# smarterclayton/kubernetes

Measured on AMD Instinct MI355X. Metric: pods scheduled/sec, higher is better.
Workload: dtype int64; 1 GPU; config2: 5000 nodes, 1776000 pods, DefaultProvider; nodes=5000, prefix_pods=0, placed_in_prefix=0, parallelism=speculative windows: all-CU snapshot scoring + in-order exact resolver

## Files before the change

### kubernetes_amd/csrc/ksg_plain.hip

```cpp
#include "ksg_launch.h"
#include "ksg_resolver.h"
#include "ksg_score.h"

#define KSG_NCAND 6
#define KSG_CSV_MAX 10
#define KSG_NO_CAND 7u
#define KSG_CSNAP 10
#define KSG_XR_W 20
#ifndef KSG_PL_PROD_SLEEP
#define KSG_PL_PROD_SLEEP 1
#endif
#ifndef KSG_PL_CHK_SLEEP
#define KSG_PL_CHK_SLEEP 2
#endif
#ifndef KSG_PL_XN_SLEEP
#define KSG_PL_XN_SLEEP 0
#endif
__host__ __device__ constexpr uint32_t pl_nt(int P) { return P >= 32 ? 512u : 768u; }
#define KSG_PL_FW KSG_RES_P0
#define KSG_PL_P0 (KSG_PL_FW + 1)
__host__ __device__ constexpr bool pl_d1(uint32_t P) { return P <= 4; }

struct alignas(16) PlCommit {
  uint32_t kind;
  uint32_t slot;
  uint32_t node;
  uint32_t flags;
  int32_t out;
  uint32_t xn;
  uint32_t pad[2];
};
struct alignas(16) PlCtl {
  uint32_t stop;
  uint32_t resolved;
  uint32_t sel_seq;
  uint32_t n_peer;
  uint32_t chk_seq[KSG_RES_NCHK];
  uint32_t chk_cnt[KSG_RES_NCHK][2];
  uint32_t chk_msk[KSG_RES_NCHK][2][2];
  uint32_t fin[KSG_RES_NCHK];
  uint32_t hang;
  uint32_t bad;
  uint32_t xseq;
  uint32_t xres[2];
  uint32_t xn_seq;
  uint32_t fin_x;
  uint32_t t_x, t_n;
  uint32_t fseq;
  uint32_t fin_f;
  uint32_t chk_rmsk[KSG_RES_NCHK][2][2];
  uint32_t chk_jmsk[KSG_RES_NCHK][2][2];
  uint32_t chk_nmsk[KSG_RES_NCHK][2][2];
  int32_t xsig[2];
};
struct PlLdsOff {
  uint32_t ctl, r_hdr, r_t0, r_wp, r_lp, r_rec, r_mod, r_svc, r_cand, r_csnap, r_csv, r_d1;
  uint32_t clist, xrow, dpos, sig, cm, peer, pub, drw, flag, peerset;
  uint32_t total;
};

__host__ __device__ inline PlLdsOff plain_lds_offsets(uint32_t P, uint32_t nflag, uint32_t W) {
  PlLdsOff o;
  const uint32_t R = win2_ring(P, false);
  uint32_t at = 0;
  o.ctl = at;     at += win_al16(sizeof(PlCtl));
  o.r_hdr = at;   at += win_al16((size_t)R * sizeof(RingHdr));
  o.r_t0 = at;    at += win_al16((size_t)R * P * 64 * 8);
  o.r_wp = at;    at += win_al16((size_t)R * P * 64 * 2);
  o.r_lp = at;    at += win_al16((size_t)R * 32 * 8);
  o.r_rec = at;   at += win_al16((size_t)R * KSG_WIN_SUM_DWORDS * 4);
  o.r_mod = at;   at += win_al16((size_t)R * 64 * 4);
  o.r_svc = at;   at += win_al16((size_t)R * sizeof(RingSvc));
  o.r_cand = at;  at += win_al16((size_t)R * 8 * 4);
  o.r_csnap = at; at += win_al16((size_t)R * KSG_NCAND * KSG_CSNAP * 8);
  o.r_csv = at;   at += win_al16((size_t)R * KSG_NCAND * KSG_SLOT_SVCS * 4);
  o.r_d1 = at;    at += pl_d1(P) ? win_al16((size_t)R * P * 64 * 8) : 0u;
  o.clist = at;   at += win_al16((size_t)KSG_MAX_SLOTS * KSG_CL_W * 4);
  o.xrow = at;    at += win_al16((size_t)KSG_MAX_SLOTS * KSG_XR_W * 4);
  o.dpos = at;    at += win_al16((size_t)2 * KSG_MAX_SLOTS * 4);
  o.sig = at;     at += win_al16((size_t)2 * KSG_MAX_SLOTS * 4);
  o.cm = at;      at += win_al16((size_t)W * sizeof(PlCommit));
  o.peer = at;    at += win_al16((size_t)win_peer_cap(nflag, W) * 2 * 4);
  o.pub = at;     at += win_al16((size_t)((W + 31) / 32) * 4);
  o.drw = at;     at += win_al16((size_t)((W + 31) / 32) * 4);
  o.flag = at;    at += win_al16((size_t)nflag * 4);
// ... 192 lines not shown
  for (int k = 0; k < 8; ++k) s += (uint32_t)__builtin_amdgcn_readlane((int)v, k);
  return s >= fused_group_arrivals(g, nwg, (uint32_t)pl_pg(P));
}

template <int P, bool STAMP, bool XS, bool FUSED>
__device__ __forceinline__ void win_plain_body(const KsgDev d, uint32_t wcap, KsgWinRun* run,
                                               const KsgWinSum* __restrict__ sums, const KsgWinXchg x,
                                               uint64_t* rng_io, int32_t* __restrict__ out_batch, const KsgFused f) {
  extern __shared__ __attribute__((aligned(16))) char smem[];
  uint32_t t_blk0 = 0;
  if constexpr (FUSED) {
    if (blockIdx.x != 0) {
      fused_score_blocks<P, STAMP>(d, wcap, run, sums, x, f, smem);
      return;
    }
    if constexpr (STAMP) t_blk0 = (uint32_t)__builtin_amdgcn_s_memrealtime();
  }
  KsgWinRun* const run_out = FUSED ? f.run_out : run;
  const uint32_t pos = run->pos, n_batch = run->n;
  if (run->halt || pos >= n_batch) {
    if (FUSED && threadIdx.x == 0) *run_out = *run;
    return;
  }
  if (FUSED && STAMP && threadIdx.x == 0 && d.dbgbuf)
    __hip_atomic_store(d.dbgbuf + 55, (int32_t)t_blk0, __ATOMIC_RELAXED, __HIP_MEMORY_SCOPE_AGENT);
  const uint32_t n_pods = min(wcap, n_batch - pos);
  int32_t* __restrict__ out = out_batch + pos;
  const uint32_t tid = threadIdx.x;
  const uint32_t lane = tid & 63;
  const uint32_t wave = __builtin_amdgcn_readfirstlane(tid >> 6);
  const uint32_t nflag = (d.n_services + 31) / 32;
  constexpr uint32_t RING = win2_ring(P, false);
  constexpr uint32_t NT = pl_nt(P);
  constexpr uint32_t NPW = NT / 64 - KSG_PL_P0;
  const uint32_t f_nwg = FUSED ? (d.nwords + NT / 64 - 1) / (NT / 64) : 0u;
  constexpr uint32_t DW = KSG_WIN_SUM_DWORDS;
  const PlLdsOff o = plain_lds_offsets(P, nflag, wcap);
  PlCtl* ctl = reinterpret_cast<PlCtl*>(smem + o.ctl);
  RingHdr* r_hdr = reinterpret_cast<RingHdr*>(smem + o.r_hdr);
  uint64_t* r_t0 = reinterpret_cast<uint64_t*>(smem + o.r_t0);
  uint64_t* r_d1 = reinterpret_cast<uint64_t*>(smem + o.r_d1);
  uint16_t* r_wp = reinterpret_cast<uint16_t*>(smem + o.r_wp);
  uint32_t* r_lp = reinterpret_cast<uint32_t*>(smem + o.r_lp);
  uint32_t* r_rec = reinterpret_cast<uint32_t*>(smem + o.r_rec);
  uint32_t* r_mod = reinterpret_cast<uint32_t*>(smem + o.r_mod);
  RingSvc* r_svc = reinterpret_cast<RingSvc*>(smem + o.r_svc);
  uint32_t* r_cand = reinterpret_cast<uint32_t*>(smem + o.r_cand);
  uint64_t* r_csnap = reinterpret_cast<uint64_t*>(smem + o.r_csnap);
  int32_t* r_csv = reinterpret_cast<int32_t*>(smem + o.r_csv);
  PlCommit* L_cm = reinterpret_cast<PlCommit*>(smem + o.cm);
  uint32_t* L_peer = reinterpret_cast<uint32_t*>(smem + o.peer);
  uint32_t* L_flag = reinterpret_cast<uint32_t*>(smem + o.flag);
  uint32_t* L_peerset = reinterpret_cast<uint32_t*>(smem + o.peerset);
  uint32_t* L_pub = reinterpret_cast<uint32_t*>(smem + o.pub);
  uint32_t* L_drw = reinterpret_cast<uint32_t*>(smem + o.drw);
  uint32_t* L_cl = reinterpret_cast<uint32_t*>(smem + o.clist);
  uint32_t* L_xr = reinterpret_cast<uint32_t*>(smem + o.xrow);
  uint32_t* L_dpos = reinterpret_cast<uint32_t*>(smem + o.dpos);
  int32_t* L_sig = reinterpret_cast<int32_t*>(smem + o.sig);
  const bool spread_on = d.w_spread != 0;
  const bool aff_on = (d.preds & KSG_PRED_SERVICEAFFINITY) && d.n_aff > 0;
  const bool res_on = (d.preds & KSG_PRED_PODFITSRESOURCES) != 0;
  const bool ports_on = (d.preds & KSG_PRED_PODFITSPORTS) != 0;
  const bool disk_on = (d.preds & KSG_PRED_NODISKCONFLICT) != 0;
  const bool xs_on = XS && (d.ext_filters & KSG_EXT_SCALAR) && d.n_scalar > 0;
  const bool esc = XS && x.esc != 0;
  const uint32_t nbits = (wcap + 31) / 32;
  const uint32_t skew = STAMP ? ((uint32_t)d.dbg >> 16) & 15u : 0u;
  const uint32_t xpt = STAMP ? ((uint32_t)d.dbg >> 24) & 15u : 0u;

  for (uint32_t t = tid; t < RING; t += NT) r_hdr[t].ready = 0;
  if (tid == 0) *ctl = PlCtl{};
  if constexpr (FUSED)
    for (uint32_t t = tid; t < f.ngroups * 8u; t += NT) st_mut(f.cnt + (size_t)(f.set ^ 1u) * f.ngroups * 8u + t, 0u);
  for (uint32_t w = tid; w < nflag; w += NT) {
    L_flag[w] = 0;
    L_peerset[w] = 0;
  }
  for (uint32_t w = tid; w < nbits; w += NT) {
    L_pub[w] = 0;
    L_drw[w] = 0;
  }
  __syncthreads();
  const uint64_t rng0 = *rng_io;

  if (wave >= KSG_PL_P0) {
    const uint32_t* recs = reinterpret_cast<const uint32_t*>(sums);
    uint64_t p_last = 0, p_acc = 0;
    auto pstamp = [&](uint32_t k) {
      if constexpr (STAMP) {
        const uint64_t t_now = __builtin_amdgcn_s_memtime();
        p_acc += lane == k ? t_now - p_last : 0ULL;
        p_last = t_now;
      }
    };
    if constexpr (STAMP) p_last = __builtin_amdgcn_s_memtime();
    const uint64_t f_t0 = (STAMP && FUSED) ? __builtin_amdgcn_s_memrealtime() : 0ULL;
    uint64_t f_tg = 0;
    for (uint32_t j = wave - KSG_PL_P0; j < n_pods; j += NPW) {
      const uint32_t e = j % RING;
      for (uint32_t spin = 0;; ++spin) {
        if (ld_acq(&ctl->stop)) return;
        if (spin > KSG_SPIN_LIMIT) {
          ctl->hang = 1;
          return;
        }
        uint32_t done = min(ld_acq(&ctl->xseq), ld_acq(&ctl->fseq) + 2u);
#pragma unroll
        for (int c = 0; c < KSG_RES_NCHK; ++c) done = min(done, ld_acq(&ctl->chk_seq[c]));
        if (j < RING || done + RING >= j + 3) break;
        __builtin_amdgcn_s_sleep(KSG_PL_PROD_SLEEP);
      }
      pstamp(24);
      if (skew & 8u) __builtin_amdgcn_s_sleep(8);
      uint32_t rec, lpv, k0;
      int32_t m0;
      if constexpr (FUSED) {
        const uint32_t g = j / (uint32_t)pl_pg(P);
        const uint32_t g_lo = (j > 0 && j % (uint32_t)pl_pg(P) == 0) ? g - 1u : g;
        for (uint32_t spin = 0;; ++spin) {
          if (ld_acq(&ctl->stop)) return;
          if (spin > KSG_SPIN_LIMIT) {
            ctl->hang = 1;
            return;
          }
          if (fused_group_done<P>(f, g, f_nwg) && (g_lo == g || fused_group_done<P>(f, g_lo, f_nwg))) break;
          __builtin_amdgcn_s_sleep(1);
        }
        rec = lane < DW ? ld_mut(recs + (size_t)j * DW + lane) : 0u;
        const int32_t* pm = reinterpret_cast<const int32_t*>(x.buf + (size_t)x.wcap * x.ostride * 8) + (size_t)j * x.ostride;
        const uint64_t* pb = reinterpret_cast<const uint64_t*>(x.buf) + (size_t)j * x.ostride;
        const uint64_t* pd = reinterpret_cast<const uint64_t*>(x.buf + x.d1_off) + (size_t)j * x.ostride;
        int32_t mw[P];
        int32_t lm = KSG_S32_NONE;
        constexpr bool ONE = P <= 8;
        uint64_t b1[ONE ? P : 1];
#pragma unroll
        for (uint32_t q = 0; q < P; ++q) {
          const uint32_t wq = q * 64 + lane;
          mw[q] = wq < d.nwords ? ld_mut(pm + wq) : KSG_S32_NONE;
          if constexpr (ONE) b1[q] = wq < d.nwords ? ld_mut(pb + wq) : 0ULL;
          lm = mw[q] > lm ? mw[q] : lm;
        }
// ... 208 lines not shown
      const bool h_prev_s = h_d1 && pod_has_service(h_prv, h_s);
      const uint32_t h_pfl = (drawable ? 0u : 1u) | (h_prev_s ? 2u : 0u) | (h_over ? 4u : 0u) | (min(nk, 255u) << 8) |
                             (min(n_svcs, 255u) << 16) | (min(n_sel, 255u) << 24);
      if (lane == 0) {
        r_hdr[e].ps = h_s;
        r_hdr[e].pfl = h_pfl;
        r_hdr[e].psoft = e_ps;
        r_hdr[e].tmax = e_tm;
        r_hdr[e].tcnt = e_tc;
        r_hdr[e].m0 = m0;
        r_hdr[e].k0 = k0;
        r_hdr[e].r = r;
        r_hdr[e].drawable = drawable;
        r_hdr[e].pred = (int32_t)cand0;
        r_hdr[e].pad = csv_on ? 1u : 0u;
        st_rel(&r_hdr[e].ready, j + 1);
      }
      if constexpr (STAMP && FUSED) {
        if (j == 0 && lane == 0 && d.dbgbuf) {
          const uint64_t t_r = __builtin_amdgcn_s_memrealtime();
          atomicAdd(d.dbgbuf + 52, (int32_t)(f_tg - f_t0));
          atomicAdd(d.dbgbuf + 53, (int32_t)(t_r - f_tg));
          atomicAdd(d.dbgbuf + 54, 1);
        }
      }
      pstamp(27);
    }
    if constexpr (STAMP) {
      if (d.dbgbuf && lane >= 24 && lane < 28) atomicAdd(d.dbgbuf + lane, (int32_t)(p_acc / 64));
    }
    return;
  }

  if (wave >= KSG_RES_C0 && wave < KSG_RES_C0 + KSG_RES_NCHK) {
    __builtin_amdgcn_s_setprio(2);
    const uint32_t c = wave - KSG_RES_C0;
    const uint32_t my_slot = c * 64 + lane;
    const uint32_t* my_cl = L_cl + (size_t)my_slot * KSG_CL_W;
    RegSlot S;
    S.node = ~0u;
    S.cap_c = S.cap_m = S.snp_c = S.snp_m = S.dl_c = S.dl_m = 0;
    S.inv_c = S.inv_m = 0.0;
    S.nk = S.ns = S.smask = 0;
    S.row = ~0u;
    S.xk = 0;
    S.sst = 0;
    S.ntm = 0;
#pragma unroll
    for (int r = 0; r < 4; ++r) S.xh[r] = S.xdl[r] = 0;
    auto apply_v = [&](uint32_t p, uint4 cmv, uint32_t prec_v) {
      const uint32_t kind = __builtin_amdgcn_readfirstlane(cmv.x);
      const uint32_t slot = __builtin_amdgcn_readfirstlane(cmv.y);
      if (kind != 1 || (slot >> 6) != c) return;
      const uint32_t woff = __builtin_amdgcn_readfirstlane(cmv.z);
      const uint32_t fl = __builtin_amdgcn_readfirstlane(cmv.w);
      const bool fresh = (fl & 1u) != 0;
      const uint32_t cidx = (fl >> 1) & 7u, n_svcs = (fl >> 8) & 0xffu, bns = (fl >> 16) & 0xffu, bnk = fl >> 24;
      const uint32_t ol = slot & 63, ep = p % RING, wn = d.lo + woff;
      const uint32_t prec = lane < DW ? prec_v : 0u;
      const PodView ppv = pod_view(prec);
      if (fresh && lane == ol) {
        if (cidx < KSG_NCAND) {
          const uint64_t* cs = r_csnap + (ep * KSG_NCAND + cidx) * KSG_CSNAP;
          S.cap_c = (int64_t)cs[0];
          S.cap_m = (int64_t)cs[1];
          S.snp_c = (int64_t)cs[2];
          S.snp_m = (int64_t)cs[3];
          S.inv_c = __longlong_as_double((long long)cs[4]);
          S.inv_m = __longlong_as_double((long long)cs[5]);
// ... 31 lines not shown
        const bool staged = cidx < KSG_NCAND && r_hdr[ep].pad != 0;
        int32_t cnt = 0;
        if (sv_lane)
          cnt = staged ? r_csv[(ep * KSG_NCAND + cidx) * KSG_SLOT_SVCS + lane] : gld(d.svc_cnt + (size_t)sv * d.n_nodes + wn);
        if (sv_lane) L_cl[(size_t)slot * KSG_CL_W + KSG_CL_SC + bns + lane] = (uint32_t)cnt;
        new_mask = wave_or_u32(sv_lane ? (1u << (sv & 31)) : 0u);
      }
      if (lane == ol) {
        S.dl_c = (int64_t)((uint64_t)S.dl_c + (uint64_t)ppv.req_c);
        S.dl_m = (int64_t)((uint64_t)S.dl_m + (uint64_t)ppv.req_m);
        S.nk = bnk + ppv.nk;
        S.ns = bns + n_svcs;
        S.smask |= new_mask;
        if (XS) {
          S.xk |= ppv.xm;
#pragma unroll
          for (int r = 0; r < 4; ++r) S.xdl[r] += (int32_t)__builtin_amdgcn_readlane(prec, WS_XREQ + r);
        }
      }
    };
    auto apply = [&](uint32_t p) {
      apply_v(p, *reinterpret_cast<const uint4*>(&L_cm[p]), r_rec[(p % RING) * DW + min(lane, DW - 1)]);
    };

    uint64_t t_last = 0, t_acc = 0;
    auto cstamp = [&](uint32_t k) {
      if constexpr (STAMP) {
        const uint64_t t_now = __builtin_amdgcn_s_memtime();
        t_acc += lane == k ? t_now - t_last : 0ULL;
        t_last = t_now;
      }
    };
    if constexpr (STAMP) t_last = __builtin_amdgcn_s_memtime();
    for (uint32_t i = 0;; ++i) {
      const uint32_t e = i % RING, par = i & 1;
      bool stopped = false;
      for (uint32_t spin = 0;; ++spin) {
        const uint32_t ss = ld_rlx(&ctl->sel_seq), rd = ld_rlx(&r_hdr[e].ready), st = ld_rlx(&ctl->stop);
        if (i < n_pods && ss + 1 >= i && rd == i + 1) break;
        if (st) {
          stopped = true;
          break;
        }
        if (spin > 16 * KSG_SPIN_LIMIT) {
          ctl->hang = 1;
          stopped = true;
          break;
        }
        if (KSG_PL_CHK_SLEEP) __builtin_amdgcn_s_sleep(KSG_PL_CHK_SLEEP);
      }
      acq_lds();
      cstamp(c == 0 ? 16 : 19);
      if (stopped) {
        const uint32_t R = __builtin_amdgcn_readfirstlane(ctl->resolved);
        for (uint32_t q = i >= 2 ? i - 2 : 0; q < R; ++q) apply(q);
        break;
      }
      if (skew & 4u) __builtin_amdgcn_s_sleep(8);
      if (xpt & 2u) {
        if (lane == 0) {
          ctl->chk_cnt[c][par] = 0;
          ctl->chk_msk[c][par][0] = ctl->chk_msk[c][par][1] = 0;
          st_post(&ctl->chk_seq[c], i + 1);
        }
        continue;
      }
      if (i >= 2) apply(i - 2);
      cstamp(c == 0 ? 17 : 20);
      const uint32_t rec = lane < DW ? r_rec[e * DW + lane] : 0u;
      const int32_t m0 = (int32_t)__builtin_amdgcn_readfirstlane(r_hdr[e].m0);
      uint64_t e_fw = 0;
      int32_t e_cs = 0;
      if (esc && S.node != ~0u) {
        e_fw = gld(efit_word(x, i, S.node >> 6));
        const int32_t ps = (int32_t)__builtin_amdgcn_readfirstlane(r_rec[e * DW + WS_SVC]);
        if (spread_on && ps >= 0) e_cs = gld(d.svc_cnt + (size_t)ps * d.n_nodes + d.lo + S.node);
      }
      bool drop = false;
      uint32_t dpos = 0;
      uint32_t est = 0;
      int32_t esig = 0;
      if (!__builtin_amdgcn_readlane(rec, WS_ERR) && m0 != KSG_S32_NONE && S.node != ~0u) {
        const PodView pv = pod_view(rec);
        const uint32_t wd = S.node >> 6;
        const uint64_t tw = r_t0[(size_t)e * P * 64 + wd];
        SlotRow R;
        R.load(my_cl);
        dpos = r_lp[e * 64 + (wd >> 6) * 2] + r_wp[(size_t)e * P * 64 + wd] +
               (uint32_t)__popcll(tw & ((1ULL << (S.node & 63)) - 1ULL));
        cstamp(c == 0 ? 22 : 40);
        if (esc) {
          const bool in_t0 = (tw >> (S.node & 63)) & 1ULL;
          const int64_t now_c = (int64_t)((uint64_t)S.snp_c + (uint64_t)S.dl_c);
          const int64_t now_m = (int64_t)((uint64_t)S.snp_m + (uint64_t)S.dl_m);
          bool unfit = false;
          if (res_on && !pv.zero_req)
            unfit = !((S.cap_c == 0 || S.cap_c - now_c >= pv.req_c) && (S.cap_m == 0 || S.cap_m - now_m >= pv.req_m));
          if (S.xk & pv.xm)
#pragma unroll
            for (int r = 0; r < 4; ++r) {
// ... 57 lines not shown
            const int32_t lr_snap =
                lr_win_nb(S.snp_c + pv.req_c, S.cap_c, S.inv_c) + lr_win_nb(S.snp_m + pv.req_m, S.cap_m, S.inv_m);
            drop |= (lr_now >> 1) != (lr_snap >> 1);
          }
          cstamp(c == 0 ? 23 : 40);
          if (!drop && pv.nk && S.nk)
            drop |= R.key_hit(S.nk, rec, pv.nk, pv.n_ports, ports_on, disk_on);
          if (!drop && spread_on && pv.s >= 0 && ((S.smask >> (pv.s & 31)) & 1u)) {
            int32_t delta = 0, snapc = 0;
            R.svc(S.ns, (uint32_t)pv.s, snapc, delta);
            if (delta)
              drop = frac10_i32(pv.smax - snapc - delta, pv.smax) != frac10_i32(pv.smax - snapc, pv.smax);
          }
        }
      }
      if (drop || (est & 4u)) L_dpos[par * KSG_MAX_SLOTS + my_slot] = dpos;
      if (est & 2u) L_sig[par * KSG_MAX_SLOTS + my_slot] = esig;
      const uint64_t dmsk = __ballot(drop);
      if (esc) {
        const uint64_t rm = __ballot((est & 2u) != 0), jm = __ballot((est & 4u) != 0), nm = __ballot((est & 8u) != 0);
        if (lane == 0) {
          ctl->chk_rmsk[c][par][0] = (uint32_t)rm;
          ctl->chk_rmsk[c][par][1] = (uint32_t)(rm >> 32);
          ctl->chk_jmsk[c][par][0] = (uint32_t)jm;
          ctl->chk_jmsk[c][par][1] = (uint32_t)(jm >> 32);
          ctl->chk_nmsk[c][par][0] = (uint32_t)nm;
          ctl->chk_nmsk[c][par][1] = (uint32_t)(nm >> 32);
        }
      }
      if (lane == 0) {
        ctl->chk_cnt[c][par] = (uint32_t)__popcll(dmsk);
        ctl->chk_msk[c][par][0] = (uint32_t)dmsk;
        ctl->chk_msk[c][par][1] = (uint32_t)(dmsk >> 32);
        st_post(&ctl->chk_seq[c], i + 1);
      }
      cstamp(c == 0 ? 18 : 21);
    }
    if (S.node != ~0u) {
      const uint32_t n = d.lo + S.node;
      d.used_cpu[n] = (int64_t)((uint64_t)S.snp_c + (uint64_t)S.dl_c);
      d.used_mem[n] = (int64_t)((uint64_t)S.snp_m + (uint64_t)S.dl_m);
      for (uint32_t a = 0; a < S.nk; ++a)
        __hip_atomic_fetch_or(d.keymap + (size_t)my_cl[KSG_CL_KEY + a] * d.nw + (n >> 6), 1ULL << (n & 63),
                              __ATOMIC_RELAXED, __HIP_MEMORY_SCOPE_AGENT);
      for (uint32_t a = 0; a < S.ns; ++a) {
        const uint32_t sa = my_cl[KSG_CL_SV + a];
        bool first = true;
        int32_t count = 0;
        for (uint32_t b = 0; b < S.ns; ++b) {
          if (my_cl[KSG_CL_SV + b] == sa) {
            if (b < a) first = false;
            ++count;
          }
        }
        __hip_atomic_fetch_add(d.svc_total + sa, 1, __ATOMIC_RELAXED, __HIP_MEMORY_SCOPE_AGENT);
        if (first) {
          const int32_t fin = (int32_t)my_cl[KSG_CL_SC + a] + count;
          d.svc_cnt[(size_t)sa * d.n_nodes + n] = fin;
          if (fin > 0)
            __hip_atomic_fetch_or(d.svc_bits + (size_t)sa * d.nw + (n >> 6), 1ULL << (n & 63), __ATOMIC_RELAXED,
                                  __HIP_MEMORY_SCOPE_AGENT);
          __hip_atomic_fetch_max(d.svc_max + sa, fin, __ATOMIC_RELAXED, __HIP_MEMORY_SCOPE_AGENT);
        }
      }
    }
    if constexpr (STAMP) {
      if (d.dbgbuf && ((lane >= 16 && lane < 24) || lane == 9 || lane == 14 || lane == 15))
        atomicAdd(d.dbgbuf + lane, (int32_t)(t_acc / 64));
    }
    drain_stores();
    if (lane == 0) st_rel(&ctl->fin[c], 1u);
    return;
  }

  auto flags = [&](uint32_t q, uint32_t node, uint32_t cidx, uint32_t slot, uint32_t bns, uint32_t prec) {
    const uint32_t nss = __builtin_amdgcn_readlane(prec, WS_NSS), npp = __builtin_amdgcn_readlane(prec, WS_NPP);
    const uint32_t n_svcs = nss >> 16, n_sel = nss & 0xffff, pnk = (npp & 0xffff) + (npp >> 16);
    if (!n_svcs) return;
    const uint32_t wn = d.lo + node, eq = q % RING;
    const bool sv_lane = lane < n_svcs;
    const uint32_t my_sv =
        (uint32_t)__shfl((int)prec, (int)min(WS_IDS + pnk + n_sel + (sv_lane ? lane : 0u), 63u), 64);
    const bool staged = cidx < KSG_NCAND && r_hdr[eq].pad != 0;
    int32_t mx = 0, peer = 0, cnt = 0;
    if (sv_lane) {
      cnt = staged ? r_csv[(eq * KSG_NCAND + cidx) * KSG_SLOT_SVCS + lane] : gld(d.svc_cnt + (size_t)my_sv * d.n_nodes + wn);
      mx = r_svc[eq].max[lane];
      peer = r_svc[eq].peer[lane];
    }
    const uint32_t ent = lane - KSG_CL_SV < bns ? L_cl[(size_t)slot * KSG_CL_W + lane] : ~0u;
    uint32_t before = 0;
    for (uint32_t t = 0; t < n_svcs; ++t) {
      const uint32_t sv_t = (uint32_t)__builtin_amdgcn_readlane((int)my_sv, (int)t);
      const uint32_t b_t = (uint32_t)__popcll(__ballot(ent == sv_t));
      if (lane == t) before = b_t;
    }
    bool changed = sv_lane && aff_on && peer == -1 && !((L_peerset[my_sv >> 5] >> (my_sv & 31)) & 1u);
    uint64_t pm = __ballot(sv_lane && peer == -1);
    if (pm) {
      uint32_t n_peer = __builtin_amdgcn_readfirstlane(ctl->n_peer);
      while (pm) {
        const uint32_t b = __builtin_ctzll(pm);
        pm &= pm - 1;
        const uint32_t fsv = (uint32_t)__builtin_amdgcn_readlane((int)my_sv, (int)b);
        if (!((L_peerset[fsv >> 5] >> (fsv & 31)) & 1u)) {
          if (lane == 0) {
            L_peerset[fsv >> 5] |= 1u << (fsv & 31);
            L_peer[2 * n_peer] = fsv;
            L_peer[2 * n_peer + 1] = wn;
          }
          ++n_peer;
          lds_fence();
        }
      }
      if (lane == 0) ctl->n_peer = n_peer;
    }
    if (sv_lane && spread_on && cnt + (int32_t)before + 1 > mx) changed = true;
    if (changed) atomicOr(&L_flag[my_sv >> 5], 1u << (my_sv & 31));
  };
  if (wave == KSG_PL_FW) {
    auto flag_commit = [&](uint32_t q) {
      const uint4 cmv = *reinterpret_cast<const uint4*>(&L_cm[q]);
      if (__builtin_amdgcn_readfirstlane(cmv.x) != 1) return;
      const uint32_t slot = __builtin_amdgcn_readfirstlane(cmv.y), node = __builtin_amdgcn_readfirstlane(cmv.z);
      const uint32_t fl = __builtin_amdgcn_readfirstlane(cmv.w);
      const uint32_t prec = lane < DW ? r_rec[(q % RING) * DW + lane] : 0u;
      flags(q, node, (fl >> 1) & 7u, slot, (fl >> 16) & 0xffu, prec);
    };
    uint64_t f_last = 0, f_acc = 0;
    auto fstamp = [&](uint32_t k) {
      if constexpr (STAMP) {
        const uint64_t t_now = __builtin_amdgcn_s_memtime();
        f_acc += lane == k ? t_now - f_last : 0ULL;
        f_last = t_now;
      }
    };
    if constexpr (STAMP) f_last = __builtin_amdgcn_s_memtime();
    uint32_t q = 0;
    for (;; ++q) {
      bool stopped = false;
      for (uint32_t spin = 0;; ++spin) {
        const uint32_t ss = ld_u(&ctl->sel_seq), st = ld_u(&ctl->stop);
        if (ss > q) break;
        if (st) {
          stopped = true;
          break;
        }
        if (spin > 16 * KSG_SPIN_LIMIT) {
          ctl->hang = 1;
          stopped = true;
          break;
        }
        __builtin_amdgcn_s_sleep(1);
// ... 502 lines not shown
    const bool x_fast = d1_on && have_x && x_fresh && !(pfl & 2u);
    if (KSG_UNLIKELY(pfl & 4u)) {
      resolved = i;
      reason = i == 0 ? KSG_STOP_OVERSIZE : KSG_STOP_SLOT;
      break;
    }
    KSG_STAMPP(1)
    struct Verd {
      uint32_t cc0, cc1, xres, fw, m0l, m0h, m1l, m1h, dp0, dp1, esw;
    };
    const uint32_t* esp = lane < 4    ? &ctl->chk_rmsk[lane >> 1][par][lane & 1]
                          : lane < 8  ? &ctl->chk_jmsk[(lane - 4) >> 1][par][lane & 1]
                          : lane < 12 ? &ctl->chk_nmsk[(lane - 8) >> 1][par][lane & 1]
                                      : reinterpret_cast<const uint32_t*>(&r_hdr[e].tcnt);
    auto verdict_reads = [&]() -> Verd {
      Verd v;
      v.cc0 = ctl->chk_cnt[0][par];
      v.cc1 = ctl->chk_cnt[1][par];
      v.xres = ctl->xres[par];
      v.fw = L_flag[(s >= 0 ? (uint32_t)s : 0u) >> 5];
      v.m0l = ctl->chk_msk[0][par][0];
      v.m0h = ctl->chk_msk[0][par][1];
      v.m1l = ctl->chk_msk[1][par][0];
      v.m1h = ctl->chk_msk[1][par][1];
      v.dp0 = L_dpos[par * KSG_MAX_SLOTS + lane];
      v.dp1 = L_dpos[par * KSG_MAX_SLOTS + 64 + lane];
      v.esw = esc ? *esp : 0u;
      return v;
    };
    bool hung = false;
    Verd vd;
    for (uint32_t spin = 0;; ++spin) {
      const uint32_t xs = ld_rlx(&ctl->xseq), hg = ld_rlx(&ctl->hang), fs = ld_rlx(&ctl->fseq);
      uint32_t cs = ld_rlx(&ctl->chk_seq[0]);
#pragma unroll
      for (int c = 1; c < KSG_RES_NCHK; ++c) cs = min(cs, ld_rlx(&ctl->chk_seq[c]));
      asm volatile("" ::: "memory");
      vd = verdict_reads();
      asm volatile("" ::"v"(vd.cc0), "v"(vd.cc1), "v"(vd.xres), "v"(vd.fw), "v"(vd.m0l), "v"(vd.m0h), "v"(vd.m1l),
                   "v"(vd.m1h), "v"(vd.dp0), "v"(vd.dp1), "v"(vd.esw));
      if ((cs >= i + 1 && (x_fast || xs >= i + 1) && fs + 1 >= i) || (xpt & 8u)) break;
      if (KSG_UNLIKELY(spin > 16 * KSG_SPIN_LIMIT || hg)) {
        hung = true;
        break;
      }
    }
    if (KSG_UNLIKELY(hung)) {
      resolved = i;
      reason = KSG_STOP_HANG;
      break;
    }
    KSG_STAMPP(2)
    if constexpr (STAMP) t_acc += lane == 6 ? (uint64_t)(uint32_t)((uint32_t)t_last - ctl->t_x) : 0ULL;
    const uint32_t cc0 = vd.cc0, cc1 = vd.cc1, fw = vd.fw;
    const uint32_t xres = x_fast ? (uint32_t)((readlane64(h.d1x, 0) >> (xnode & 63)) & 1ULL) : __builtin_amdgcn_readfirstlane(vd.xres);
    uint64_t msk0 = ((uint64_t)__builtin_amdgcn_readfirstlane(vd.m0h) << 32) | (uint32_t)__builtin_amdgcn_readfirstlane(vd.m0l);
    uint64_t msk1 = ((uint64_t)__builtin_amdgcn_readfirstlane(vd.m1h) << 32) | (uint32_t)__builtin_amdgcn_readfirstlane(vd.m1l);
    const uint32_t dp0 = vd.dp0, dp1 = vd.dp1;
    acq_lds();
    if (KSG_UNLIKELY(s >= 0 && (spread_on || aff_on) && ((xres & 2u) || ((__builtin_amdgcn_readfirstlane(fw) >> (s & 31)) & 1u)))) {
      resolved = i;
      reason = KSG_STOP_SERVICE;
      break;
    }

    const bool x_kept = !(((xslot < 64 ? msk0 : msk1) >> (xslot & 63)) & 1ULL);
    bool x_drop = have_x && (xres & 1u) && ((t0x >> (xnode & 63)) & 1ULL) && x_kept;
    uint32_t dropped = (xpt & 4u) ? 0u : __builtin_amdgcn_readfirstlane(cc0) + __builtin_amdgcn_readfirstlane(cc1) + (x_drop ? 1u : 0u);
    KSG_STAMPP(12)
// ... 204 lines not shown
      st_post(&ctl->sel_seq, i + 1);
    }
    if ((int32_t)woff != pred) KSG_COUNTP(8, 64)
    if (lane == (slot & 63)) {
      if (slot >= 64) {
        if (!in_c) cn1 = woff;
        dc1 = new_dc;
        dm1 = new_dm;
        sk1 = base_nk + nk;
        ss1 = base_ns + n_svcs;
      } else {
        if (!in_c) cn0 = woff;
        dc0 = new_dc;
        dm0 = new_dm;
        sk0 = base_nk + nk;
        ss0 = base_ns + n_svcs;
      }
    }
    have_x = true;
    xnode = woff;
    xslot = slot;
    x_fresh = !in_c;
    ++n_draws;
    KSG_STAMPP(5)
  }
  if (lane == 0) {
    ctl->resolved = resolved;
    st_rel(&ctl->stop, 1u);
  }
  bool drained = false;
  for (uint32_t spin = 0; spin <= 16 * KSG_SPIN_LIMIT; ++spin) {
    bool done = ld_acq(&ctl->fin_x) != 0 && ld_acq(&ctl->fin_f) != 0;
#pragma unroll
    for (int c = 0; c < KSG_RES_NCHK; ++c) done = done && ld_acq(&ctl->fin[c]) != 0;
    if (done) {
      drained = true;
      break;
    }
  }
  if (ld_acq(&ctl->bad)) reason = KSG_STOP_BAD;
  else if (!drained || ld_acq(&ctl->hang)) reason = KSG_STOP_HANG;
  if constexpr (STAMP) {
    if (d.dbgbuf && (lane < 16 || lane == 43 || lane == 44)) atomicAdd(d.dbgbuf + lane, (int32_t)(t_acc / 64));
  }
#undef KSG_STAMPP
#undef KSG_COUNTP
  const uint32_t n_peer = __builtin_amdgcn_readfirstlane(ctl->n_peer);
  for (uint32_t t = lane; t < n_peer; t += 64) {
    const uint32_t sv = L_peer[2 * t];
    int32_t expect = -1;
    __hip_atomic_compare_exchange_strong(d.svc_peer + sv, &expect, (int32_t)L_peer[2 * t + 1], __ATOMIC_RELAXED,
                                         __ATOMIC_RELAXED, __HIP_MEMORY_SCOPE_AGENT);
  }
  for (uint32_t t = lane; t < resolved; t += 64) out[t] = L_cm[t].out;
  if (esc && x.tmax) {
    for (uint32_t t = lane; t < wcap; t += 64) x.tmax[t] = 0;
    for (uint32_t t = lane; t < n_pods * KSG_TBINS; t += 64) x.thist[t] = 0;
  }
  if (XS) {
    for (uint32_t t = lane; t < resolved; t += 64) {
      if (L_cm[t].kind != 1) continue;
      const ksg_pod_ext& pe = x.exts[pos + t];
      const uint32_t wn = d.lo + L_cm[t].node;
      for (uint32_t r = 0; r < d.n_scalar; ++r)
        if (pe.scalar[r] != 0)
          __hip_atomic_fetch_add(reinterpret_cast<uint64_t*>(d.scalar_used + (size_t)r * d.n_nodes + wn),
                                 (uint64_t)pe.scalar[r], __ATOMIC_RELAXED, __HIP_MEMORY_SCOPE_AGENT);
// ... 164 lines not shown
```

### kubernetes_amd/csrc/ksg_resolver.h

```cpp
#pragma once
#include "ksg_device.h"

#include <algorithm>

#define WS_ERR 2
#define WS_SVC 3
#define WS_HOST 4
#define WS_SMAX 5
#define WS_STOT 6
#define WS_NINL 7
#define WS_CPU 8
#define WS_MEM 10
#define WS_AFF 12
#define WS_NPP 16
#define WS_NSS 17
#define WS_XM 18
#define WS_IDS 19
#define WS_XREQ 43

__host__ __device__ constexpr uint32_t win_res_nt(uint32_t P) { return P <= 8 ? 512u : 512u; }
#define KSG_RES_C0 2
#define KSG_RES_NCHK 2
#define KSG_RES_P0 (KSG_RES_C0 + KSG_RES_NCHK)
#define KSG_RES_NPW (KSG_RES_NT / 64 - KSG_RES_P0)
// ... 99 lines not shown
  o.r_fit = at;   at += anti && !win2_fg(P) ? win_al16((size_t)KSG_RING * P * 64 * 8) : 0u;
  o.s_meta = at;  at += win_al16((size_t)KSG_MAX_SLOTS * sizeof(SlotMeta));
  o.s_cap = at;   at += win_al16((size_t)KSG_MAX_SLOTS * sizeof(I64x2));
  o.s_snp = at;   at += win_al16((size_t)KSG_MAX_SLOTS * sizeof(I64x2));
  o.s_dl = at;    at += win_al16((size_t)KSG_MAX_SLOTS * sizeof(I64x2));
  o.s_inv = at;   at += win_al16((size_t)KSG_MAX_SLOTS * sizeof(F64x2));
  o.keys = at;    at += win_al16((size_t)KSG_MAX_SLOTS * KSG_SLOT_KEYS * 4);
  o.svcs = at;    at += win_al16((size_t)KSG_MAX_SLOTS * KSG_SLOT_SVCS * 4);
  o.scnt = at;    at += win_al16((size_t)KSG_MAX_SLOTS * KSG_SLOT_SVCS * 4);
  o.peer = at;    at += win_al16((size_t)win_peer_cap(nflag, W) * 2 * 4);
  o.out = at;     at += win_al16((size_t)W * 4);
  o.flag = at;    at += win_al16((size_t)nflag * 4);
  o.peerset = at; at += win_al16((size_t)nflag * 4);
  o.drop = at;    at += win_al16((size_t)2 * P * 64 * 8);
  o.ord = at;     at += win_al16((size_t)2 * sizeof(WinOrder));
  o.r_b = at;     at += dz ? win_al16((size_t)KSG_RING * P * 64 * 8) : 0u;
  o.r_mb = at;    at += dz ? win_al16((size_t)KSG_RING * KSG_RR_MAXZ * 4) : 0u;
  o.r_dc = at;    at += dz ? win_al16((size_t)KSG_RING * KSG_RR_MAXZ * 4) : 0u;
  o.zm = at;      at += win_al16((size_t)dz * P * 64 * 8);
  o.nsv = at;     at += dz ? win_al16((size_t)nsvc * 4) : 0u;
  o.dca = at;     at += dz ? win_al16((size_t)KSG_RES_NCHK * 2 * KSG_RR_MAXZ * 4) : 0u;
  o.total = at;
  return o;
}

#define KSG_STOP_SERVICE 1
#define KSG_STOP_EXHAUSTED 2
#define KSG_STOP_SLOT 3
#define KSG_STOP_OVERSIZE 4
#define KSG_STOP_HANG 9
#define KSG_STOP_BAD 10
#define KSG_SPIN_LIMIT (1u << 22)
#define KSG_DBG_SKEW_MASK 0x000f0000u
#define KSG_DBG_RESOLVER_MASK 0x0f0f0000u

template <typename T>
__device__ __forceinline__ T gld(const T* p) {
  return *(const __attribute__((address_space(1))) T*)p;
}
__device__ __forceinline__ void lds_fence() { __builtin_amdgcn_fence(__ATOMIC_SEQ_CST, "wavefront"); }
#define KSG_UNLIKELY(c) __builtin_expect(!!(c), 0)
__device__ __forceinline__ uint32_t ld_acq(uint32_t* p) {
  return __hip_atomic_load(p, __ATOMIC_ACQUIRE, __HIP_MEMORY_SCOPE_WORKGROUP);
}
__device__ __forceinline__ void st_rel(uint32_t* p, uint32_t v) {
  __hip_atomic_store(p, v, __ATOMIC_RELEASE, __HIP_MEMORY_SCOPE_WORKGROUP);
}
__device__ __forceinline__ void st_post(uint32_t* p, uint32_t v) {
#ifdef KSG_POST_RELEASE
  st_rel(p, v);
#else
  asm volatile("" ::: "memory");
  __hip_atomic_store(p, v, __ATOMIC_RELAXED, __HIP_MEMORY_SCOPE_WORKGROUP);
#endif
}
__device__ __forceinline__ uint32_t ld_rlx(uint32_t* p) {
  return __hip_atomic_load(p, __ATOMIC_RELAXED, __HIP_MEMORY_SCOPE_WORKGROUP);
}
__device__ __forceinline__ void acq_lds() { __builtin_amdgcn_fence(__ATOMIC_ACQUIRE, "workgroup", "local"); }
__device__ __forceinline__ uint32_t ld_u(uint32_t* p) {
  return (uint32_t)__builtin_amdgcn_readfirstlane((int)ld_rlx(p));
}

template <int P>
__device__ __forceinline__ uint32_t select_in_lanes(const uint64_t (&bits)[P], uint32_t cl, uint32_t incl,
                                                    uint32_t target, uint32_t lane) {
  const uint32_t excl = incl - cl;
// ... 242 lines not shown
```

Before: 821,500 pods/s.

## Interleave checker waves across two sets handling alternating pods

For small P, the checker stage is replicated into CS sets of waves. Each set processes every CS-th pod and catches up by applying the commits it skipped (apply(na)) while waiting. The resolver reads the per-parity checker sequence, and producers wait on all sets. This aims to halve the per-pod checker latency on the critical path, at the cost of extra waves (fewer producer waves), redundant apply work in every set, and more complex synchronisation.

Result: slower. 768,200 pods/s (-6.5%).

```diff
diff --git a/kubernetes_amd/csrc/ksg_plain.hip b/kubernetes_amd/csrc/ksg_plain.hip
--- a/kubernetes_amd/csrc/ksg_plain.hip
+++ b/kubernetes_amd/csrc/ksg_plain.hip
@@ -17,8 +17,15 @@
 #define KSG_PL_XN_SLEEP 0
 #endif
 __host__ __device__ constexpr uint32_t pl_nt(int P) { return P >= 32 ? 512u : 768u; }
-#define KSG_PL_FW KSG_RES_P0
-#define KSG_PL_P0 (KSG_PL_FW + 1)
+#define KSG_PL_C0 2u
+#define KSG_PL_NCHK 2u
+#ifndef KSG_PL_CS_SMALL
+#define KSG_PL_CS_SMALL 2u
+#endif
+__host__ __device__ constexpr uint32_t pl_cs(int P) { return P <= 8 ? KSG_PL_CS_SMALL : 1u; }
+__host__ __device__ constexpr uint32_t pl_fw(int P) { return KSG_PL_C0 + pl_cs(P) * KSG_PL_NCHK; }
+__host__ __device__ constexpr uint32_t pl_p0(int P) { return pl_fw(P) + 1u; }
+static_assert(KSG_MAX_SLOTS == 64 * KSG_PL_NCHK, "lane l of a set's wave c owns slot 64c + l");
 __host__ __device__ constexpr bool pl_d1(uint32_t P) { return P <= 4; }
 
 struct alignas(16) PlCommit {
@@ -35,10 +42,10 @@
   uint32_t resolved;
   uint32_t sel_seq;
   uint32_t n_peer;
-  uint32_t chk_seq[KSG_RES_NCHK];
-  uint32_t chk_cnt[KSG_RES_NCHK][2];
-  uint32_t chk_msk[KSG_RES_NCHK][2][2];
-  uint32_t fin[KSG_RES_NCHK];
+  uint32_t chk_seq[2][KSG_PL_NCHK];
+  uint32_t chk_cnt[KSG_PL_NCHK][2];
+  uint32_t chk_msk[KSG_PL_NCHK][2][2];
+  uint32_t fin[KSG_PL_NCHK];
   uint32_t hang;
   uint32_t bad;
   uint32_t xseq;
@@ -48,9 +55,9 @@
   uint32_t t_x, t_n;
   uint32_t fseq;
   uint32_t fin_f;
-  uint32_t chk_rmsk[KSG_RES_NCHK][2][2];
-  uint32_t chk_jmsk[KSG_RES_NCHK][2][2];
-  uint32_t chk_nmsk[KSG_RES_NCHK][2][2];
+  uint32_t chk_rmsk[KSG_PL_NCHK][2][2];
+  uint32_t chk_jmsk[KSG_PL_NCHK][2][2];
+  uint32_t chk_nmsk[KSG_PL_NCHK][2][2];
   int32_t xsig[2];
 };
 struct PlLdsOff {
@@ -309,7 +316,9 @@
   const uint32_t nflag = (d.n_services + 31) / 32;
   constexpr uint32_t RING = win2_ring(P, false);
   constexpr uint32_t NT = pl_nt(P);
-  constexpr uint32_t NPW = NT / 64 - KSG_PL_P0;
+  constexpr uint32_t CS = pl_cs(P);
+  constexpr uint32_t PL_FW = pl_fw(P), PL_P0 = pl_p0(P);
+  constexpr uint32_t NPW = NT / 64 - PL_P0;
   const uint32_t f_nwg = FUSED ? (d.nwords + NT / 64 - 1) / (NT / 64) : 0u;
   constexpr uint32_t DW = KSG_WIN_SUM_DWORDS;
   const PlLdsOff o = plain_lds_offsets(P, nflag, wcap);
@@ -343,7 +352,7 @@
   const bool xs_on = XS && (d.ext_filters & KSG_EXT_SCALAR) && d.n_scalar > 0;
   const bool esc = XS && x.esc != 0;
   const uint32_t nbits = (wcap + 31) / 32;
-  const uint32_t skew = STAMP ? ((uint32_t)d.dbg >> 16) & 15u : 0u;
+  const uint32_t skew = STAMP ? ((uint32_t)d.dbg >> 16) & 0x3fu : 0u;
   const uint32_t xpt = STAMP ? ((uint32_t)d.dbg >> 24) & 15u : 0u;
 
   for (uint32_t t = tid; t < RING; t += NT) r_hdr[t].ready = 0;
@@ -361,7 +370,7 @@
   __syncthreads();
   const uint64_t rng0 = *rng_io;
 
-  if (wave >= KSG_PL_P0) {
+  if (wave >= PL_P0) {
     const uint32_t* recs = reinterpret_cast<const uint32_t*>(sums);
     uint64_t p_last = 0, p_acc = 0;
     auto pstamp = [&](uint32_t k) {
@@ -374,7 +383,7 @@
     if constexpr (STAMP) p_last = __builtin_amdgcn_s_memtime();
     const uint64_t f_t0 = (STAMP && FUSED) ? __builtin_amdgcn_s_memrealtime() : 0ULL;
     uint64_t f_tg = 0;
-    for (uint32_t j = wave - KSG_PL_P0; j < n_pods; j += NPW) {
+    for (uint32_t j = wave - PL_P0; j < n_pods; j += NPW) {
       const uint32_t e = j % RING;
       for (uint32_t spin = 0;; ++spin) {
         if (ld_acq(&ctl->stop)) return;
@@ -384,8 +393,9 @@
         }
         uint32_t done = min(ld_acq(&ctl->xseq), ld_acq(&ctl->fseq) + 2u);
 #pragma unroll
-        for (int c = 0; c < KSG_RES_NCHK; ++c) done = min(done, ld_acq(&ctl->chk_seq[c]));
-        if (j < RING || done + RING >= j + 3) break;
+        for (uint32_t sc = 0; sc < CS * KSG_PL_NCHK; ++sc)
+          done = min(done, ld_acq(&ctl->chk_seq[sc / KSG_PL_NCHK][sc % KSG_PL_NCHK]));
+        if (j < RING || done + RING >= j + 2 + CS) break;
         __builtin_amdgcn_s_sleep(KSG_PL_PROD_SLEEP);
       }
       pstamp(24);
@@ -660,9 +670,10 @@
     return;
   }
 
-  if (wave >= KSG_RES_C0 && wave < KSG_RES_C0 + KSG_RES_NCHK) {
+  if (wave >= KSG_PL_C0 && wave < PL_FW) {
     __builtin_amdgcn_s_setprio(2);
-    const uint32_t c = wave - KSG_RES_C0;
+    const uint32_t cset = (wave - KSG_PL_C0) / KSG_PL_NCHK;
+    const uint32_t c = (wave - KSG_PL_C0) % KSG_PL_NCHK;
     const uint32_t my_slot = c * 64 + lane;
     const uint32_t* my_cl = L_cl + (size_t)my_slot * KSG_CL_W;
     RegSlot S;
@@ -760,12 +771,22 @@
       }
     };
     if constexpr (STAMP) t_last = __builtin_amdgcn_s_memtime();
-    for (uint32_t i = 0;; ++i) {
+    const bool skewed = (skew & 4u) || (skew & (16u << cset));
+    uint32_t na = 0;
+    for (uint32_t i = cset;; i += CS) {
       const uint32_t e = i % RING, par = i & 1;
       bool stopped = false;
       for (uint32_t spin = 0;; ++spin) {
         const uint32_t ss = ld_rlx(&ctl->sel_seq), rd = ld_rlx(&r_hdr[e].ready), st = ld_rlx(&ctl->stop);
         if (i < n_pods && ss + 1 >= i && rd == i + 1) break;
+        if (CS > 1 && na + 2 < i && ss > na && !(xpt & 2u)) {
+          acq_lds();
+          cstamp(c == 0 ? 16 : 19);
+          apply(na);
+          ++na;
+          cstamp(c == 0 ? 17 : 20);
+          continue;
+        }
         if (st) {
           stopped = true;
           break;
@@ -781,19 +802,20 @@
       cstamp(c == 0 ? 16 : 19);
       if (stopped) {
         const uint32_t R = __builtin_amdgcn_readfirstlane(ctl->resolved);
-        for (uint32_t q = i >= 2 ? i - 2 : 0; q < R; ++q) apply(q);
+        for (; na < R; ++na) apply(na);
         break;
       }
-      if (skew & 4u) __builtin_amdgcn_s_sleep(8);
+      if (skewed) __builtin_amdgcn_s_sleep(8);
       if (xpt & 2u) {
         if (lane == 0) {
           ctl->chk_cnt[c][par] = 0;
           ctl->chk_msk[c][par][0] = ctl->chk_msk[c][par][1] = 0;
-          st_post(&ctl->chk_seq[c], i + 1);
-        }
+          st_post(&ctl->chk_seq[cset][c], i + 1);
+        }
+        if (i >= 2) na = i - 1;
         continue;
       }
-      if (i >= 2) apply(i - 2);
+      for (; na + 2 <= i; ++na) apply(na);
       cstamp(c == 0 ? 17 : 20);
       const uint32_t rec = lane < DW ? r_rec[e * DW + lane] : 0u;
       const int32_t m0 = (int32_t)__builtin_amdgcn_readfirstlane(r_hdr[e].m0);
@@ -917,10 +939,15 @@
         ctl->chk_cnt[c][par] = (uint32_t)__popcll(dmsk);
         ctl->chk_msk[c][par][0] = (uint32_t)dmsk;
         ctl->chk_msk[c][par][1] = (uint32_t)(dmsk >> 32);
-        st_post(&ctl->chk_seq[c], i + 1);
+        st_post(&ctl->chk_seq[cset][c], i + 1);
       }
       cstamp(c == 0 ? 18 : 21);
     }
+    if constexpr (STAMP) {
+      if (d.dbgbuf && ((lane >= 16 && lane < 24) || lane == 9 || lane == 14 || lane == 15))
+        atomicAdd(d.dbgbuf + lane, (int32_t)(t_acc / 64));
+    }
+    if (cset != 0) return;
     if (S.node != ~0u) {
       const uint32_t n = d.lo + S.node;
       d.used_cpu[n] = (int64_t)((uint64_t)S.snp_c + (uint64_t)S.dl_c);
@@ -949,10 +976,6 @@
         }
       }
     }
-    if constexpr (STAMP) {
-      if (d.dbgbuf && ((lane >= 16 && lane < 24) || lane == 9 || lane == 14 || lane == 15))
-        atomicAdd(d.dbgbuf + lane, (int32_t)(t_acc / 64));
-    }
     drain_stores();
     if (lane == 0) st_rel(&ctl->fin[c], 1u);
     return;
@@ -1003,7 +1026,7 @@
     if (sv_lane && spread_on && cnt + (int32_t)before + 1 > mx) changed = true;
     if (changed) atomicOr(&L_flag[my_sv >> 5], 1u << (my_sv & 31));
   };
-  if (wave == KSG_PL_FW) {
+  if (wave == PL_FW) {
     auto flag_commit = [&](uint32_t q) {
       const uint4 cmv = *reinterpret_cast<const uint4*>(&L_cm[q]);
       if (__builtin_amdgcn_readfirstlane(cmv.x) != 1) return;
@@ -1572,9 +1595,10 @@
     Verd vd;
     for (uint32_t spin = 0;; ++spin) {
       const uint32_t xs = ld_rlx(&ctl->xseq), hg = ld_rlx(&ctl->hang), fs = ld_rlx(&ctl->fseq);
-      uint32_t cs = ld_rlx(&ctl->chk_seq[0]);
-#pragma unroll
-      for (int c = 1; c < KSG_RES_NCHK; ++c) cs = min(cs, ld_rlx(&ctl->chk_seq[c]));
+      uint32_t* const cw = ctl->chk_seq[CS > 1 ? par : 0u];
+      uint32_t cs = ld_rlx(&cw[0]);
+#pragma unroll
+      for (uint32_t c = 1; c < KSG_PL_NCHK; ++c) cs = min(cs, ld_rlx(&cw[c]));
       asm volatile("" ::: "memory");
       vd = verdict_reads();
       asm volatile("" ::"v"(vd.cc0), "v"(vd.cc1), "v"(vd.xres), "v"(vd.fw), "v"(vd.m0l), "v"(vd.m0h), "v"(vd.m1l),
@@ -1845,7 +1869,7 @@
   for (uint32_t spin = 0; spin <= 16 * KSG_SPIN_LIMIT; ++spin) {
     bool done = ld_acq(&ctl->fin_x) != 0 && ld_acq(&ctl->fin_f) != 0;
 #pragma unroll
-    for (int c = 0; c < KSG_RES_NCHK; ++c) done = done && ld_acq(&ctl->fin[c]) != 0;
+    for (uint32_t c = 0; c < KSG_PL_NCHK; ++c) done = done && ld_acq(&ctl->fin[c]) != 0;
     if (done) {
       drained = true;
       break;
diff --git a/kubernetes_amd/csrc/ksg_resolver.h b/kubernetes_amd/csrc/ksg_resolver.h
--- a/kubernetes_amd/csrc/ksg_resolver.h
+++ b/kubernetes_amd/csrc/ksg_resolver.h
@@ -155,7 +155,7 @@
 #define KSG_STOP_BAD 10
 #define KSG_SPIN_LIMIT (1u << 22)
 #define KSG_DBG_SKEW_MASK 0x000f0000u
-#define KSG_DBG_RESOLVER_MASK 0x0f0f0000u
+#define KSG_DBG_RESOLVER_MASK 0x0f3f0000u
 
 template <typename T>
 __device__ __forceinline__ T gld(const T* p) {
```
